# UCL/gp_emulator

Hardware: AMD Instinct MI355X
Metric: test-points/sec for predict(mean+var+grad), N_train=250 D=11 (higher is better)
Workload: dtype f64

## Files before the change

### gp_emulator_amd/csrc/gp_predict_few_kernel.hpp

```cpp
#pragma once
#include "gp_predict_kernel.hpp"

namespace gpk {

constexpr int fkWaves = 8;
constexpr int fkThreads = fkWaves * 64;
constexpr int fkMaxKSteps = 4 * 20;

template <typename T, int D, bool kVar = true>
__global__ __launch_bounds__(fkThreads, 2) void predict_few_kernel(PredictArgs<T> p, int NB) {
  typedef Real<T> R;
  typedef typename R::acc_t acc_t;
  constexpr int DS = row_stride(D);
  constexpr int kVals = D + 2;

  __shared__ __attribute__((aligned(16))) T s_xa[4 * fkMaxKSteps * row_stride(D)];
  __shared__ T s_k[kVar ? fkMaxKSteps : 1][64];
  __shared__ T s_part[fkWaves][kTile][kVals];

  const int tid = threadIdx.x;
  const int lane = tid & 63;
  const int w = __builtin_amdgcn_readfirstlane(tid >> 6);
  const int ml = lane & 15, g = lane >> 4;
  const int n_tiles = (int)((p.M + kTile - 1) / kTile);
  const int e = blockIdx.x / n_tiles, tile = blockIdx.x - e * n_tiles;
  const int NKS = 4 * NB;

  const T* xa = p.xa + e * p.xa_stride;
  const T* frags = p.frags + e * p.frags_stride;
  (void)frags;
  const T* sdp = p.sd + e * p.sd_stride;
  const long long m = (long long)tile * kTile + ml;
  const long long mc = m < p.M ? m : p.M - 1;

  {
    const int n = 16 * NB * DS;
#pragma unroll 4
    for (int i = tid; i < n; i += fkThreads) s_xa[i] = xa[i];
  }

  T t[D];
  T gm = T(0);
#pragma unroll
  for (int d = 0; d < D; ++d) {
    const bool live = d < p.d_actual;
    const int dc = live ? d : p.d_actual - 1;
    const T sc = !live ? T(0) : p.rows_prescaled ? T(1) : sdp[d];
    const T ce = (!live || p.rows_prescaled) ? T(0) : sdp[D + d];
    t[d] = sc * (p.testing[mc * p.d_actual + dc] - ce);
    gm = fma(t[d], t[d], gm);
  }
  gm *= T(-0.5);
  const T poison = gm - gm;
  const T b = sdp[2 * D];
  __syncthreads();

  T mu = T(0);
  T ga[D];
#pragma unroll
  for (int d = 0; d < D; ++d) ga[d] = T(0);
#pragma unroll 1
  for (int ks = w; ks < NKS; ks += fkWaves) {
    const int i = own_index<T>(ks >> 2, ks & 3, g);
    const T* row = &s_xa[i * DS];
    T x[D];
#pragma unroll
    for (int d = 0; d < D; ++d) x[d] = row[d];
    const T al = row[D];
    T k;
    if constexpr (R::kExpand) {
      k = row[D + 1] + gm;
#pragma unroll
      for (int d = 0; d < D; ++d) k = fma(x[d], t[d], k);
      k = R::exp_clamped(k);
    } else {
      T r2 = T(0);
#pragma unroll
      for (int d = 0; d < D; ++d) {
        x[d] -= t[d];
        r2 = fma(x[d], x[d], r2);
      }
      k = b * R::exp_clamped(T(-0.5) * r2);
    }
    if constexpr (kVar) s_k[ks][lane] = k;
    const T wgt = k * al;
    mu += wgt;
#pragma unroll
    for (int d = 0; d < D; ++d) ga[d] = fma(wgt, x[d], ga[d]);
  }
  mu = xor_reduce_groups(mu);
  xor_reduce_groups_n<T, D>(ga);
  if (g == 0) {
    s_part[w][ml][0] = mu;
#pragma unroll
    for (int d = 0; d < D; ++d) s_part[w][ml][1 + d] = ga[d];
  }
  __syncthreads();

  if constexpr (kVar) {
  T vacc = T(0);
  auto column_block = [&](const int J) __attribute__((always_inline)) {
    const T* f = frags + ((size_t)frag_index(J, J, 0, NB) * 64 + lane);
    const int n = 4 * (NB - J);
    acc_t acc = acc_t{T(0), T(0), T(0), T(0)};
    T a_cur[4], a_nxt[4];
#pragma unroll
    for (int s = 0; s < 4; ++s) a_cur[s] = f[(size_t)s * 64];
#pragma unroll 1
    for (int q = 0; q < n; q += 4) {
      const int qn = q + 4 < n ? q + 4 : q;
#pragma unroll
      for (int s = 0; s < 4; ++s) a_nxt[s] = f[(size_t)(qn + s) * 64];
#pragma unroll
      for (int s = 0; s < 4; ++s) acc = R::mfma(a_cur[s], s_k[4 * J + q + s][lane], acc);
#pragma unroll
      for (int s = 0; s < 4; ++s) a_cur[s] = a_nxt[s];
    }
#pragma unroll
    for (int r = 0; r < 4; ++r) vacc = fma(acc[r], s_k[4 * J + r][lane], vacc);
  };
  for (int pr = w; 2 * pr < NB; pr += fkWaves) {
    column_block(pr);
    if (NB - 1 - pr != pr) column_block(NB - 1 - pr);
  }
  vacc = xor_reduce_groups(vacc);
  if (g == 0) s_part[w][ml][1 + D] = vacc;
  __syncthreads();
  }

  if (w == 0 && m < p.M) {
    auto total = [&](const int v) __attribute__((always_inline)) {
      T s = s_part[0][ml][v];
#pragma unroll
      for (int k = 1; k < fkWaves; ++k) s += s_part[k][ml][v];
      return s;
    };
    const T mean = total(0) + poison;
    T* o_mu = p.mu + e * p.M;
    T* o_der = p.deriv + e * p.M * p.d_actual;
    if (g == 0) o_mu[m] = mean;
    if constexpr (kVar) {
      if (g == 1) p.var[e * p.M + m] = b - total(1 + D) + poison;
    }
#pragma unroll
    for (int d = 0; d < D; ++d) {
      if ((d & 3) == g && d < p.d_actual) {
        const T gsum = total(1 + d);
        const T gd = sdp[d] * (R::kExpand ? fma(-t[d], mean, gsum) : gsum + poison);
        if (p.deriv_row_major) o_der[m * p.d_actual + d] = gd;
        else o_der[(long long)d * p.M + m] = gd;
      }
    }
  }
}

}
```

### gp_emulator_amd/csrc/gp_predict_kernel.hpp

```cpp
#pragma once
#include <hip/hip_runtime.h>
#include <stdint.h>
#include <type_traits>
#include <utility>

namespace gpk {

#ifndef GP_WAVES
#define GP_WAVES 8
#endif
#ifndef GP_WAVES_F32
#define GP_WAVES_F32 12
#endif
#ifndef GP_CHUNK
#define GP_CHUNK 64
#endif
#ifndef GP_CHUNK_F32
#define GP_CHUNK_F32 192
#endif
#ifndef GP_ABLATE
#define GP_ABLATE 0
#endif
#ifndef GP_AHEAD
#define GP_AHEAD 4
#endif
#ifndef GP_AHEAD_F32
#define GP_AHEAD_F32 8
#endif
#ifndef GP_RING_PIN
#define GP_RING_PIN 1
#endif
#ifndef GP_MU_DOUBLE
#define GP_MU_DOUBLE 1
#endif
#ifndef GP_ESTRIN
#define GP_ESTRIN 0
#endif
#ifndef GP_EXP_FUSED
#define GP_EXP_FUSED 1
#endif
#ifndef GP_DOTSPLIT
#define GP_DOTSPLIT 1
#endif
#ifndef GP_GROUP_F64
#define GP_GROUP_F64 1
#endif
#ifndef GP_STAMPS
#define GP_STAMPS 0
#endif
constexpr int kTile = 16;
template <typename T, bool kVar = true> struct Geo {
  static constexpr int kWaves = sizeof(T) == 8 ? GP_WAVES : GP_WAVES_F32;
  static constexpr int kThreads = kWaves * 64;
#ifndef GP_WG_PER_CU_SMALL
#define GP_WG_PER_CU_SMALL 0
#endif
  static constexpr int kWGPerCU = kWaves >= 8 ? 1 : (GP_WG_PER_CU_SMALL > 0 ? GP_WG_PER_CU_SMALL : 8 / kWaves);
  static constexpr int kWavesPerSimd = kWaves >= 8 ? kWaves / 4 : kWGPerCU * kWaves / 4;
  static constexpr int kRowsPerWG = kWaves * kTile;
  static constexpr int kChunk = sizeof(T) == 8 ? GP_CHUNK : GP_CHUNK_F32;
};
#ifndef GP_MG_WAVES
#define GP_MG_WAVES 12
#endif
#ifndef GP_MG_WAVES_F32
#define GP_MG_WAVES_F32 16
#endif
#ifndef GP_MG_WG_PER_CU
#define GP_MG_WG_PER_CU 1
#endif
template <typename T> struct Geo<T, false> {
  static constexpr int kWaves = sizeof(T) == 8 ? GP_MG_WAVES : GP_MG_WAVES_F32;
  static constexpr int kThreads = kWaves * 64;
  static constexpr int kWGPerCU = GP_MG_WG_PER_CU;
  static constexpr int kWavesPerSimd = kWGPerCU * kWaves / 4;
  static constexpr int kRowsPerWG = kWaves * kTile;
  static constexpr int kChunk = 1;
};

typedef double f64x4 __attribute__((ext_vector_type(4)));
typedef float f32x4 __attribute__((ext_vector_type(4)));

template <typename F, int... Is>
__device__ __forceinline__ void static_for_impl(F&& f, std::integer_sequence<int, Is...>) {
  (f(std::integral_constant<int, Is>{}), ...);
}
template <int N, typename F>
__device__ __forceinline__ void static_for(F&& f) {
  static_for_impl(f, std::make_integer_sequence<int, N>{});
}

template <typename T> struct Real;
template <> struct Real<double> {
  typedef f64x4 acc_t;
  static constexpr bool kExpand = true;
  static constexpr int kGroup = GP_GROUP_F64;
  __host__ __device__ static constexpr int own_sub(int r, int g) { return 4 * r + g; }
  __device__ static inline acc_t mfma(double a, double b, acc_t c) {
    return __builtin_amdgcn_mfma_f64_16x16x4f64(a, b, c, 0, 0, 0);
  }
  static constexpr double kRoundMagic = 6755399441055744.0;
  __host__ __device__ static inline double exp_(double x) {
#if GP_EXP_FUSED
    const double s = fma(x, 1.4426950408889634, kRoundMagic);
    const double n = s - kRoundMagic;
    const int ni = (int)(unsigned)__builtin_bit_cast(unsigned long long, s);
#else
    x = __builtin_fmax(x, -1000.0);
    const double n = __builtin_rint(x * 1.4426950408889634);
    const int ni = (int)n;
#endif
    double r = fma(n, -6.93147180559945286e-01, x);
    r = fma(n, -2.31904681384629956e-17, r);
#if GP_ESTRIN
    const double r2 = r * r;
    const double p01 = fma(1.00000000000000666e+00, r, 1.0);
    const double p23 = fma(1.66666666665544028e-01, r, 5.00000000000000555e-01);
    const double p45 = fma(8.33333338566834801e-03, r, 4.16666666665732183e-02);
    const double p67 = fma(1.98411702695461072e-04, r, 1.38888889324666632e-03);
    const double p89 = fma(2.76401812311866076e-06, r, 2.48015043709117912e-05);
    const double r4 = r2 * r2;
    const double q0 = fma(r2, p23, p01);
    const double q1 = fma(r2, p67, p45);
    const double q2 = fma(r2, 2.76263485910095559e-07, p89);
    const double r8 = r4 * r4;
    const double s0 = fma(r4, q1, q0);
    const double p = fma(r8, q2, s0);
#else
    double p = 2.76263485910095559e-07;
    p = fma(p, r, 2.76401812311866076e-06);
    p = fma(p, r, 2.48015043709117912e-05);
    p = fma(p, r, 1.98411702695461072e-04);
    p = fma(p, r, 1.38888889324666632e-03);
    p = fma(p, r, 8.33333338566834801e-03);
    p = fma(p, r, 4.16666666665732183e-02);
    p = fma(p, r, 1.66666666665544028e-01);
    p = fma(p, r, 5.00000000000000555e-01);
    p = fma(p, r, 1.00000000000000666e+00);
    p = fma(p, r, 1.0);
#endif
    return ldexp(p, ni);
  }
  __host__ __device__ static inline double exp_clamped(double x) { return exp_(__builtin_fmax(x, -1000.0)); }
  template <int GP>
  __device__ static inline void exp_n(double (&x)[GP]) {
    double n[GP], r[GP], p[GP];
    int ni[GP];
#pragma unroll
    for (int u = 0; u < GP; ++u) x[u] = __builtin_fmax(x[u], -1000.0);
#if GP_EXP_FUSED
#pragma unroll
    for (int u = 0; u < GP; ++u) r[u] = fma(x[u], 1.4426950408889634, kRoundMagic);
#pragma unroll
    for (int u = 0; u < GP; ++u) {
      n[u] = r[u] - kRoundMagic;
      ni[u] = (int)(unsigned)__builtin_bit_cast(unsigned long long, r[u]);
    }
#else
#pragma unroll
    for (int u = 0; u < GP; ++u) {
      n[u] = __builtin_rint(x[u] * 1.4426950408889634);
      ni[u] = (int)n[u];
    }
#endif
#pragma unroll
    for (int u = 0; u < GP; ++u) r[u] = fma(n[u], -6.93147180559945286e-01, x[u]);
#pragma unroll
    for (int u = 0; u < GP; ++u) r[u] = fma(n[u], -2.31904681384629956e-17, r[u]);
#pragma unroll
    for (int u = 0; u < GP; ++u) p[u] = 2.76263485910095559e-07;
    constexpr double c[10] = {2.76401812311866076e-06, 2.48015043709117912e-05, 1.98411702695461072e-04,
                              1.38888889324666632e-03, 8.33333338566834801e-03, 4.16666666665732183e-02,
                              1.66666666665544028e-01, 5.00000000000000555e-01, 1.00000000000000666e+00, 1.0};
#pragma unroll
    for (int j = 0; j < 10; ++j) {
#pragma unroll
      for (int u = 0; u < GP; ++u) p[u] = fma(p[u], r[u], c[j]);
    }
#pragma unroll
    for (int u = 0; u < GP; ++u) x[u] = ldexp(p[u], ni[u]);
  }
  static constexpr double kMaxHalfNorm2 = 67108864.0;
  static constexpr double kFarG = 134217728.0;
};
template <> struct Real<float> {
  typedef f32x4 acc_t;
  static constexpr bool kExpand = false;
#ifndef GP_GROUP_F32
#define GP_GROUP_F32 2
#endif
  static constexpr int kGroup = GP_GROUP_F32;
  __host__ __device__ static constexpr int own_sub(int r, int g) { return 4 * g + r; }
  __device__ static inline acc_t mfma(float a, float b, acc_t c) {
    return __builtin_amdgcn_mfma_f32_16x16x4f32(a, b, c, 0, 0, 0);
  }
  __device__ static inline float exp_(float x) { return __expf(x); }
  __device__ static inline float exp_clamped(float x) { return __expf(x); }
  template <int GP>
  __device__ static inline void exp_n(float (&x)[GP]) {
#pragma unroll
    for (int u = 0; u < GP; ++u) x[u] = __expf(x[u]);
  }
};

template <typename T>
__host__ __device__ constexpr int own_index(int I, int s, int g) {
  return 16 * I + Real<T>::own_sub(s, g);
}

template <typename T>
__host__ __device__ constexpr int point_slot(int n) {
  return 16 * (n / 16) + Real<T>::own_sub((n % 16) / 4, n % 4);
}
template <typename T>
__host__ __device__ constexpr int slot_point(int slot) {
  for (int q = 0; q < 16; ++q)
    if (Real<T>::own_sub(q / 4, q % 4) == slot % 16) return 16 * (slot / 16) + q;
  return -1;
}

struct FragId { int I, J, s; };
__host__ __device__ constexpr int frag_count(int NB) { return NB * (NB + 1) / 2 * 4; }
__host__ __device__ constexpr int frag_col_offset(int J, int NB) { return J * NB - J * (J - 1) / 2; }
__host__ __device__ constexpr FragId frag_at(int n, int NB) {
  const int pair = n >> 2;
  int J = 0;
  while (J + 1 < NB && frag_col_offset(J + 1, NB) <= pair) ++J;
  return FragId{J + pair - frag_col_offset(J, NB), J, n & 3};
}
__host__ __device__ constexpr int frag_index(int I, int J, int s, int NB) {
  return (frag_col_offset(J, NB) + (I - J)) * 4 + s;
}
__host__ __device__ constexpr int frag_count_padded(int NB, int chunk) {
  return (frag_count(NB) + chunk - 1) / chunk * chunk;
}

__host__ __device__ constexpr int row_stride(int D) { return (D + 2 + 3) & ~3; }
#ifndef GP_XA_PAD
#define GP_XA_PAD 1
#endif
template <typename T> __host__ __device__ constexpr int xa_lds_stride(int D) {
  return (GP_XA_PAD && sizeof(T) == 4 && row_stride(D) % 16 == 0) ? row_stride(D) + 4 : row_stride(D);
}

#ifndef GP_FRAG_BUFS
#define GP_FRAG_BUFS 3
#endif
#ifndef GP_FRAG_BUFS_F32
#define GP_FRAG_BUFS_F32 2
#endif
#ifndef GP_SEAM
#define GP_SEAM 2
#endif
constexpr int kLdsBudget = 160 * 1024;
constexpr int kLdsSlack = 32;
template <typename T>
__host__ __device__ constexpr int predict_lds_bytes(int D, int NK, int bufs) {
  const int NP = 16 * ((NK + 3) / 4);
  return (int)sizeof(T) * (NP * xa_lds_stride<T>(D) + bufs * Geo<T>::kChunk * 64 + (2 * D + 1) + 2 * D +
                           2 * Geo<T>::kWaves * kTile * D) + kLdsSlack;
}
template <typename T>
__host__ __device__ constexpr int frag_buffers(int D, int NK) {
  const int want = sizeof(T) == 8 ? GP_FRAG_BUFS : GP_FRAG_BUFS_F32;
  return want > 2 && predict_lds_bytes<T>(D, NK, want) <= kLdsBudget ? want : 2;
}

template <typename T>
struct PredictArgs {
  const T* xa;
  const T* frags;
  const T* sd;
  const T* testing;
  T* mu;
  T* var;
  T* deriv;
  long long M;
  int d_actual;
  int deriv_row_major;
  int n_emulators;
  long long xa_stride, frags_stride, sd_stride;
  unsigned long long* dbg;
  int rows_prescaled;
};

template <int XOR>
__device__ __forceinline__ unsigned swap_halves(unsigned x, unsigned& other) {
  if constexpr (XOR == 16) {
    auto r = __builtin_amdgcn_permlane16_swap(x, x, false, false);
    other = r[1];
    return r[0];
  } else {
    auto r = __builtin_amdgcn_permlane32_swap(x, x, false, false);
    other = r[1];
    return r[0];
  }
}
template <int XOR>
__device__ __forceinline__ float pair_sum(float v) {
  unsigned o, a = swap_halves<XOR>(__float_as_uint(v), o);
  return __uint_as_float(a) + __uint_as_float(o);
}
template <int XOR>
__device__ __forceinline__ double pair_sum(double v) {
  const unsigned long long u = (unsigned long long)__double_as_longlong(v);
  unsigned lo_o, hi_o;
  const unsigned lo_a = swap_halves<XOR>((unsigned)u, lo_o);
  const unsigned hi_a = swap_halves<XOR>((unsigned)(u >> 32), hi_o);
  const double a = __longlong_as_double((long long)(((unsigned long long)hi_a << 32) | lo_a));
  const double o = __longlong_as_double((long long)(((unsigned long long)hi_o << 32) | lo_o));
  return a + o;
}

template <typename T, int N>
__device__ inline void xor_reduce_groups_n(T* v) {
#pragma unroll
  for (int i = 0; i < N; ++i) v[i] = pair_sum<32>(pair_sum<16>(v[i]));
}

template <typename T>
__device__ inline T xor_reduce_groups(T v) {
  return pair_sum<32>(pair_sum<16>(v));
}

template <typename T, int kWaves = Geo<T>::kWaves, int kChunk = Geo<T>::kChunk>
__device__ __forceinline__ void stage_chunk(const T* src, T* dst, int wave, int lane) {
  constexpr int kBytes = kChunk * 64 * (int)sizeof(T);
  constexpr int kPieces = kBytes / 1024;
  static_assert(kPieces * 1024 == kBytes, "chunk must be whole 1 KiB pieces");
  const unsigned voff = (unsigned)lane * 16u;
  const unsigned lds0 = (unsigned)(uintptr_t)(
      (__attribute__((address_space(3))) char*)(reinterpret_cast<char*>(dst)));
#pragma unroll
  for (int pc0 = 0; pc0 < kPieces; pc0 += kWaves) {
    const int pc = pc0 + wave;
    if (pc0 + kWaves <= kPieces || pc < kPieces) {
      const char* s = reinterpret_cast<const char*>(src) + pc * 1024;
      const unsigned m0v = __builtin_amdgcn_readfirstlane(lds0 + pc * 1024);
      unsigned keep;
      asm volatile(
          "s_mov_b32 %0, m0\n\t"
          "s_mov_b32 m0, %1\n\t"
          "s_nop 4\n\t"
          "global_load_lds_dwordx4 %2, %3\n\t"
          "s_mov_b32 m0, %0"
          : "=&s"(keep)
          : "s"(m0v), "v"(voff), "s"(s)
          : "memory");
    }
  }
}
template <typename T, int NP>
__device__ __forceinline__ void stage_pieces(const T* src, T* dst, int first_piece, int lane) {
  const unsigned voff = (unsigned)lane * 16u;
  const unsigned lds0 = (unsigned)(uintptr_t)(
      (__attribute__((address_space(3))) char*)(reinterpret_cast<char*>(dst)));
#pragma unroll
  for (int i = 0; i < NP; ++i) {
    const int pc = first_piece + i;
    const char* s = reinterpret_cast<const char*>(src) + pc * 1024;
    const unsigned m0v = __builtin_amdgcn_readfirstlane(lds0 + pc * 1024);
    unsigned keep;
    asm volatile(
        "s_mov_b32 %0, m0\n\t"
        "s_mov_b32 m0, %1\n\t"
        "s_nop 4\n\t"
        "global_load_lds_dwordx4 %2, %3\n\t"
        "s_mov_b32 m0, %0"
        : "=&s"(keep)
        : "s"(m0v), "v"(voff), "s"(s)
        : "memory");
  }
}
__device__ __forceinline__ void dma_wait() { asm volatile("s_waitcnt vmcnt(0)" ::: "memory"); }

#if GP_STAMPS == 1
#define GP_STAMP(seg)                                                                    \
  do {                                                                                   \
    __builtin_amdgcn_sched_barrier(0);                                                   \
    unsigned long long now_;                                                             \
    asm volatile("s_memtime %0\n\ts_waitcnt lgkmcnt(0)" : "=s"(now_)::"memory");         \
    __builtin_amdgcn_sched_barrier(0);                                                   \
    seg_sum[seg] += now_ - seg_t0;                                                       \
    seg_t0 = now_;                                                                       \
  } while (0)
#else
#define GP_STAMP(seg) do { } while (0)
#endif

template <typename T, int D, int NK, bool kVar = true>
__global__ __launch_bounds__((Geo<T, kVar>::kThreads), (Geo<T, kVar>::kWavesPerSimd)) void predict_kernel(PredictArgs<T> p) {
  typedef Real<T> R;
  typedef Geo<T, kVar> G;
  constexpr int kThreads = G::kThreads;
  constexpr int kRowsPerWG = G::kRowsPerWG;
  typedef typename R::acc_t acc_t;
  constexpr int NB = (NK + 3) / 4;
  constexpr int KL = NK - 4 * (NB - 1);
  constexpr int NP = 16 * NB;
  constexpr int DSG = row_stride(D);
  constexpr int DS = xa_lds_stride<T>(D);
  constexpr int NF = frag_count(NB);
  constexpr int kChunk = G::kChunk;
  constexpr int NCH = (NF + kChunk - 1) / kChunk;
  constexpr int kBufs = kVar ? frag_buffers<T>(D, NK) : 1;
  constexpr int kLook = kBufs - 2;
  constexpr bool kSeamOk = kVar && kBufs == 3 && NCH >= 3 && NCH % 3 == 0;
  constexpr bool kSeamAblated = (GP_ABLATE == 5 || GP_ABLATE == 6) && kSeamOk;
  constexpr bool kSeam = GP_SEAM && !kSeamAblated && kSeamOk;
  constexpr bool kSeamTop = kSeam || kSeamAblated;
  constexpr bool kSeamAlways = kSeam && GP_SEAM == 2;

  __shared__ __attribute__((aligned(16))) T s_xa[NP * DS];
  __shared__ __attribute__((aligned(16))) T s_fr[kBufs][kVar ? kChunk * 64 : 1];
  __shared__ T s_sd[2 * D + 1];
  __shared__ T s_ts[2 * D];
  __shared__ T s_rows[2][G::kWaves][kTile * D];
  static_assert(!kVar || (int)(sizeof(s_xa) + sizeof(s_fr) + sizeof(s_sd) + sizeof(s_ts) + sizeof(s_rows)) + kLdsSlack ==
                             predict_lds_bytes<T>(D, NK, kBufs), "predict_lds_bytes() does not count the kernel's LDS arrays");

  const int tid = threadIdx.x;
  const int lane = tid & 63;
  const int wave = __builtin_amdgcn_readfirstlane(tid >> 6);
  const int ml = lane & 15;
  const int g = lane >> 4;

  const int n_groups = (int)((p.M + kRowsPerWG - 1) / kRowsPerWG);
  int e = 0, cur_e = -1;
  int grp = blockIdx.x;
  while (grp >= n_groups && e < p.n_emulators) { grp -= n_groups; ++e; }

  constexpr int NJ = (kTile * D + 63) / 64;
  auto fetch_rows = [&](int grp_, T (&regs)[NJ]) {
    const long long e0 = ((long long)grp_ * kRowsPerWG + wave * kTile) * p.d_actual;
    const long long emax = p.M * p.d_actual - 1;
#pragma unroll
    for (int j = 0; j < NJ; ++j) {
      long long e_ = e0 + lane + 64 * j;
      e_ = e_ < emax ? e_ : emax;
      regs[j] = p.testing[e_];
    }
  };
  auto stash_rows = [&](int buf_, const T (&regs)[NJ]) {
#pragma unroll
    for (int j = 0; j < NJ; ++j) asm volatile("" ::"v"(regs[j]));
#pragma unroll
    for (int j = 0; j < NJ; ++j)
      if (lane + 64 * j < kTile * p.d_actual) s_rows[buf_][wave][lane + 64 * j] = regs[j];
  };
  int rbuf = 0;
  T rregs[NJ];
  if (e < p.n_emulators) {
    fetch_rows(grp, rregs);
    stash_rows(0, rregs);
  }
#if GP_STAMPS
  unsigned long long seg_sum[8] = {0, 0, 0, 0, 0, 0, 0, 0};
  unsigned long long seg_t0;
  asm volatile("s_memtime %0\n\ts_waitcnt lgkmcnt(0)" : "=s"(seg_t0)::"memory");
#endif

  for (; e < p.n_emulators;) {
    const T* frags = p.frags + e * p.frags_stride;
    auto open_ring = [&]() {
      __syncthreads();
      static_for<1 + kLook>([&](auto cc) {
        constexpr int c = decltype(cc)::value;
        if constexpr (c < NCH) stage_chunk<T, G::kWaves, kChunk>(frags + c * kChunk * 64, &s_fr[c][0], wave, lane);
      });
    };
    if (e != cur_e) {
      cur_e = e;
      if constexpr (kSeamAlways) dma_wait();
      __syncthreads();
      const T* xa = p.xa + e * p.xa_stride;
      for (int i = tid; i < NP * DSG; i += kThreads) s_xa[(i / DSG) * DS + i % DSG] = xa[i];
      const T* sdp = p.sd + e * p.sd_stride;
      if (tid < 2 * D + 1) {
        const bool live = tid == 2 * D || (tid % D) < p.d_actual;
        s_sd[tid] = live ? sdp[tid] : T(0);
        if (tid < 2 * D)
          s_ts[tid] = !live ? T(0) : !p.rows_prescaled ? sdp[tid] : tid < D ? T(1) : T(0);
      }
      if constexpr (!kVar) __syncthreads();
      if constexpr (kVar && kSeamTop) open_ring();
    }
    T* o_mu = p.mu + e * p.M;
    T* o_der = p.deriv + e * p.M * p.d_actual;
    const long long m = (long long)grp * kRowsPerWG + wave * kTile + ml;
    const long long mc = m < p.M ? m : p.M - 1;

    if constexpr (kVar) {
      if constexpr (!kSeamTop) open_ring();
    } else {
      (void)frags;
      __builtin_amdgcn_fence(__ATOMIC_ACQ_REL, "wavefront");
      __builtin_amdgcn_wave_barrier();
    }
    const T b = s_sd[2 * D];
    GP_STAMP(0);

    T t[D];
    T gm = T(0);
    {
      T sdv[D], cv[D], rv[D];
#pragma unroll
      for (int d = 0; d < D; ++d) {
        const int dc = d < p.d_actual ? d : p.d_actual - 1;
        sdv[d] = s_ts[d];
        cv[d] = s_ts[D + d];
        rv[d] = s_rows[rbuf][wave][ml * p.d_actual + dc];
      }
#pragma unroll
      for (int d = 0; d < D; ++d) {
        t[d] = sdv[d] * (rv[d] - cv[d]);
        gm = fma(t[d], t[d], gm);
      }
    }
    gm *= T(-0.5);
    const T poison = gm - gm;
    if constexpr (R::kExpand && GP_EXP_FUSED) {
      const bool in_reach = gm >= T(-R::kFarG);
#pragma unroll
      for (int d = 0; d < D; ++d) t[d] = in_reach ? t[d] : T(0);
      gm = in_reach ? gm : T(-R::kFarG);
    }

    asm volatile("" :: "v"(gm));
    int e_next = e, grp_next = grp + gridDim.x;
    while (grp_next >= n_groups && e_next < p.n_emulators) { grp_next -= n_groups; ++e_next; }
    fetch_rows(e_next < p.n_emulators ? grp_next : grp, rregs);
    const bool ahead = kSeam && e_next == e;

    GP_STAMP(1);
    T kv[NK];
#if GP_MU_DOUBLE
    double mu = 0.0;
#else
    T mu = T(0);
#endif
    T ga[D];
#pragma unroll
    for (int d = 0; d < D; ++d) ga[d] = T(0);

    constexpr int GP = R::kGroup;
    static_for<(NK + GP - 1) / GP>([&](auto qc) {
      constexpr int q0 = decltype(qc)::value * GP;
      constexpr int GU = NK - q0 < GP ? NK - q0 : GP;
      T x[GP][D];
      T al[GP];
      T k[GP];
#pragma unroll
      for (int u = 0; u < GU; ++u) {
        const int q = q0 + u;
        const int i = own_index<T>(q >> 2, q & 3, g);
        const T* row = &s_xa[i * DS];
#pragma unroll
        for (int d = 0; d < D; ++d) x[u][d] = row[d];
        al[u] = row[D];
        if constexpr (R::kExpand) k[u] = row[D + 1] + gm;
      }
#pragma unroll
      for (int u = 0; u < GU; ++u) {
#if GP_ABLATE == 2
        continue;
#endif
        if constexpr (R::kExpand) {
          T part[GP_DOTSPLIT];
          part[0] = k[u];
#pragma unroll
          for (int c = 1; c < GP_DOTSPLIT; ++c) part[c] = T(0);
#pragma unroll
          for (int d = 0; d < D; ++d) part[d % GP_DOTSPLIT] = fma(x[u][d], t[d], part[d % GP_DOTSPLIT]);
#pragma unroll
          for (int c = 1; c < GP_DOTSPLIT; ++c) part[0] += part[c];
          k[u] = part[0];
        } else {
          T r2 = T(0);
#pragma unroll
          for (int d = 0; d < D; ++d) {
            x[u][d] -= t[d];
            r2 = fma(x[u][d], x[u][d], r2);
          }
          k[u] = T(-0.5) * r2;
        }
      }
#pragma unroll
      for (int u = 0; u < GU; ++u) {
#if GP_ABLATE == 2
        k[u] = x[u][0] + t[0];
#else
        k[u] = R::kExpand ? R::exp_(k[u]) : b * R::exp_(k[u]);
#endif
        if constexpr (kVar) kv[q0 + u] = k[u];
      }
#pragma unroll
      for (int u = 0; u < GU; ++u) {
        const T w = k[u] * al[u];
        mu += (decltype(mu))w;
#if GP_ABLATE == 2
        ga[u % D] += w;
#else
#pragma unroll
        for (int d = 0; d < D; ++d) ga[d] = fma(w, x[u][d], ga[d]);
#endif
      }
    });
    GP_STAMP(2);
    const T mu_t = (T)xor_reduce_groups(mu) + poison;
    static_for<(D + 5) / 6>([&](auto bc) {
      constexpr int d0 = decltype(bc)::value * 6;
      constexpr int nb_ = (D - d0 < 6) ? (D - d0) : 6;
      xor_reduce_groups_n<T, nb_>(&ga[d0]);
    });
    {
      T sdv[D];
#pragma unroll
      for (int d = 0; d < D; ++d) sdv[d] = s_sd[d];
#pragma unroll
      for (int d = 0; d < D; ++d)
        ga[d] = R::kExpand ? sdv[d] * fma(-t[d], mu_t, ga[d]) : fma(sdv[d], ga[d], poison);
    }

    if (m < p.M) {
      if (g == 0) o_mu[m] = mu_t;
      int gs = g;
      asm volatile("" : "+v"(gs));
      T gq[(D + 3) / 4];
#pragma unroll
      for (int q = 0; q < (D + 3) / 4; ++q) {
        gq[q] = ga[4 * q];
#pragma unroll
        for (int u = 1; u < 4; ++u)
          if (4 * q + u < D) gq[q] = gs == u ? ga[4 * q + u] : gq[q];
      }
      if (p.deriv_row_major) {
        T* o_row = o_der + m * p.d_actual + gs;
#pragma unroll
        for (int q = 0; q < (D + 3) / 4; ++q)
          if (4 * q + gs < p.d_actual) o_row[4 * q] = gq[q];
      } else {
        T* o_row = o_der + gs * p.M + m;
#pragma unroll
        for (int q = 0; q < (D + 3) / 4; ++q)
          if (4 * q + gs < p.d_actual) o_row[4 * q * p.M] = gq[q];
      }
    }

    GP_STAMP(3);
    stash_rows(rbuf ^ 1, rregs);
    if constexpr (!kVar) {
      rbuf ^= 1;
      e = e_next;
      grp = grp_next;
      continue;
    } else {

    T* o_var = p.var + e * p.M;
    T vacc = T(0);
    acc_t acc;
    constexpr int kAhead = sizeof(T) == 4 ? GP_AHEAD_F32 : GP_AHEAD;
    T afr[kAhead];
#if GP_ABLATE == 1
    static_for<NK>([&](auto qc) { vacc += kv[decltype(qc)::value]; });
    static_for<0>([&](auto fc) {
#else
    static_for<NF>([&](auto fc) {
#endif
      constexpr int f = decltype(fc)::value;
      constexpr int c = f / kChunk, fl = f % kChunk;
      constexpr FragId fid = frag_at(f, NB);
      constexpr int I = fid.I, J = fid.J, s = fid.s;
      if constexpr (fl == 0) {
#if GP_ABLATE == 4
        if constexpr (c == 0) { dma_wait(); __syncthreads(); }
#else
        if constexpr (c == 0 || c + kLook < NCH) {
          dma_wait();
          if constexpr (kLook > 0) {
            if constexpr (c > 0) __builtin_amdgcn_sched_barrier(0);
            asm volatile("s_barrier" ::: "memory");
            if constexpr (c > 0) __builtin_amdgcn_sched_barrier(0);
          } else {
            __syncthreads();
          }
          if constexpr (c + kLook + 1 < NCH) {
            stage_chunk<T, G::kWaves, kChunk>(frags + (c + kLook + 1) * kChunk * 64,
                                              &s_fr[(c + kLook + 1) % kBufs][0], wave, lane);
          } else if constexpr (kSeam && c == NCH - 2) {
            if (kSeamAlways || ahead) stage_chunk<T, G::kWaves, kChunk>(frags, &s_fr[0][0], wave, lane);
          }
        } else if constexpr (GP_ABLATE == 6 && kSeamAblated && c == NCH - 1) {
          __builtin_amdgcn_sched_barrier(0);
          asm volatile("s_barrier" ::: "memory");
          __builtin_amdgcn_sched_barrier(0);
        } else if constexpr (kSeam && c == NCH - 1) {
          if (kSeamAlways || ahead) {
            __builtin_amdgcn_sched_barrier(0);
            asm volatile("s_barrier" ::: "memory");
            __builtin_amdgcn_sched_barrier(0);
            stage_chunk<T, G::kWaves, kChunk>(frags + kChunk * 64, &s_fr[1][0], wave, lane);
          }
        }
#endif
        static_for<kAhead - 1>([&](auto jc) {
          constexpr int n = f + decltype(jc)::value;
          if constexpr (n < NF && (c == 0 || n / kChunk > c - 1 + kLook)) {
#if GP_ABLATE >= 3
            afr[n % kAhead] = kv[n % NK];
#else
            afr[n % kAhead] = s_fr[(n / kChunk) % kBufs][(n % kChunk) * 64 + lane];
#endif
          }
        });
      }
      {
        constexpr int n = f + kAhead - 1;
        if constexpr (n < NF && n / kChunk <= c + kLook) {
#if GP_ABLATE >= 3
          afr[n % kAhead] = kv[(f + 1) % NK];
#else
          afr[n % kAhead] = s_fr[(n / kChunk) % kBufs][(n % kChunk) * 64 + lane];
#endif
        }
      }
      if constexpr (I == J && s == 0) acc = acc_t{T(0), T(0), T(0), T(0)};
      if constexpr (4 * I + s < NK) acc = R::mfma(afr[f % kAhead], kv[4 * I + s], acc);
#if GP_RING_PIN
      if constexpr (sizeof(T) == 4 || GP_RING_PIN > 1) __builtin_amdgcn_sched_barrier(0);
#endif
      if constexpr (I == NB - 1 && s == 3) {
#pragma unroll
        for (int r = 0; r < (J == NB - 1 ? KL : 4); ++r) vacc = fma(acc[r], kv[4 * J + r], vacc);
      }
    });
    rbuf ^= 1;
    GP_STAMP(4);
    vacc = xor_reduce_groups(vacc);
    if (m < p.M && g == 1) o_var[m] = b - vacc + poison;

    e = e_next;
    grp = grp_next;
    GP_STAMP(5);
    }
  }
  if constexpr (kSeamAlways) dma_wait();
#if GP_STAMPS
  if (lane == 0 && p.dbg) {
    for (int k_ = 0; k_ < 8; ++k_) atomicAdd(&p.dbg[k_], seg_sum[k_]);
    atomicAdd(&p.dbg[7], 1ull);
  }
#endif
}

}
```

Baseline: 763.2 million.

## Interleave fragment order across column groups to use independent MFMA accumulators

```diff
diff --git a/gp_emulator_amd/csrc/gp_predict_few_kernel.hpp b/gp_emulator_amd/csrc/gp_predict_few_kernel.hpp
--- a/gp_emulator_amd/csrc/gp_predict_few_kernel.hpp
+++ b/gp_emulator_amd/csrc/gp_predict_few_kernel.hpp
@@ -100,17 +100,19 @@
   if constexpr (kVar) {
   T vacc = T(0);
   auto column_block = [&](const int J) __attribute__((always_inline)) {
-    const T* f = frags + ((size_t)frag_index(J, J, 0, NB) * 64 + lane);
+    auto frag = [&](const int I, const int s) __attribute__((always_inline)) {
+      return frags[(size_t)frag_index(I, J, s, NB) * 64 + lane];
+    };
     const int n = 4 * (NB - J);
     acc_t acc = acc_t{T(0), T(0), T(0), T(0)};
     T a_cur[4], a_nxt[4];
 #pragma unroll
-    for (int s = 0; s < 4; ++s) a_cur[s] = f[(size_t)s * 64];
+    for (int s = 0; s < 4; ++s) a_cur[s] = frag(J, s);
 #pragma unroll 1
     for (int q = 0; q < n; q += 4) {
       const int qn = q + 4 < n ? q + 4 : q;
 #pragma unroll
-      for (int s = 0; s < 4; ++s) a_nxt[s] = f[(size_t)(qn + s) * 64];
+      for (int s = 0; s < 4; ++s) a_nxt[s] = frag(J + qn / 4, s);
 #pragma unroll
       for (int s = 0; s < 4; ++s) acc = R::mfma(a_cur[s], s_k[4 * J + q + s][lane], acc);
 #pragma unroll
diff --git a/gp_emulator_amd/csrc/gp_predict_kernel.hpp b/gp_emulator_amd/csrc/gp_predict_kernel.hpp
--- a/gp_emulator_amd/csrc/gp_predict_kernel.hpp
+++ b/gp_emulator_amd/csrc/gp_predict_kernel.hpp
@@ -219,17 +219,37 @@
   return -1;
 }
 
+#ifndef GP_COLGROUP
+#define GP_COLGROUP 4
+#endif
+#if GP_ABLATE == 7
+constexpr int kColGroup = 1;
+#else
+constexpr int kColGroup = GP_COLGROUP;
+#endif
 struct FragId { int I, J, s; };
 __host__ __device__ constexpr int frag_count(int NB) { return NB * (NB + 1) / 2 * 4; }
 __host__ __device__ constexpr int frag_col_offset(int J, int NB) { return J * NB - J * (J - 1) / 2; }
+__host__ __device__ constexpr int frag_group_width(int J0, int NB) { return NB - J0 < kColGroup ? NB - J0 : kColGroup; }
+__host__ __device__ constexpr int frag_row_width(int I, int J0, int NB) {
+  return I - J0 + 1 < frag_group_width(J0, NB) ? I - J0 + 1 : frag_group_width(J0, NB);
+}
+__host__ __device__ constexpr int frag_row_offset(int I, int J0, int NB) {
+  const int d = I - J0, w = frag_group_width(J0, NB);
+  return d <= w ? d * (d + 1) / 2 : w * (w + 1) / 2 + (d - w) * w;
+}
+__host__ __device__ constexpr int frag_index(int I, int J, int s, int NB) {
+  const int J0 = J - J % kColGroup;
+  return (frag_col_offset(J0, NB) + frag_row_offset(I, J0, NB)) * 4 + s * frag_row_width(I, J0, NB) + (J - J0);
+}
 __host__ __device__ constexpr FragId frag_at(int n, int NB) {
   const int pair = n >> 2;
-  int J = 0;
-  while (J + 1 < NB && frag_col_offset(J + 1, NB) <= pair) ++J;
-  return FragId{J + pair - frag_col_offset(J, NB), J, n & 3};
-}
-__host__ __device__ constexpr int frag_index(int I, int J, int s, int NB) {
-  return (frag_col_offset(J, NB) + (I - J)) * 4 + s;
+  int J0 = 0;
+  while (J0 + kColGroup < NB && frag_col_offset(J0 + kColGroup, NB) <= pair) J0 += kColGroup;
+  int I = J0;
+  while (I + 1 < NB && frag_col_offset(J0, NB) + frag_row_offset(I + 1, J0, NB) <= pair) ++I;
+  const int r = n - (frag_col_offset(J0, NB) + frag_row_offset(I, J0, NB)) * 4, w = frag_row_width(I, J0, NB);
+  return FragId{I, J0 + r % w, r / w};
 }
 __host__ __device__ constexpr int frag_count_padded(int NB, int chunk) {
   return (frag_count(NB) + chunk - 1) / chunk * chunk;
@@ -658,7 +678,11 @@
 
     T* o_var = p.var + e * p.M;
     T vacc = T(0);
-    acc_t acc;
+    constexpr int kAcc = GP_ABLATE == 7 ? GP_COLGROUP : kColGroup;
+    acc_t acc[kAcc];
+#if GP_ABLATE == 7
+    static_for<kAcc>([&](auto ac) { acc[decltype(ac)::value] = acc_t{T(0), T(0), T(0), T(0)}; });
+#endif
     constexpr int kAhead = sizeof(T) == 4 ? GP_AHEAD_F32 : GP_AHEAD;
     T afr[kAhead];
 #if GP_ABLATE == 1
@@ -724,14 +748,27 @@
 #endif
         }
       }
-      if constexpr (I == J && s == 0) acc = acc_t{T(0), T(0), T(0), T(0)};
-      if constexpr (4 * I + s < NK) acc = R::mfma(afr[f % kAhead], kv[4 * I + s], acc);
+      constexpr int J0 = J - J % kColGroup, GW = frag_group_width(J0, NB);
+      constexpr int a = GP_ABLATE == 7 ? f % kAcc : J - J0;
+      if constexpr (I == J && s == 0) acc[a] = acc_t{T(0), T(0), T(0), T(0)};
+      if constexpr (4 * I + s < NK) acc[a] = R::mfma(afr[f % kAhead], kv[4 * I + s], acc[a]);
 #if GP_RING_PIN
       if constexpr (sizeof(T) == 4 || GP_RING_PIN > 1) __builtin_amdgcn_sched_barrier(0);
 #endif
-      if constexpr (I == NB - 1 && s == 3) {
-#pragma unroll
-        for (int r = 0; r < (J == NB - 1 ? KL : 4); ++r) vacc = fma(acc[r], kv[4 * J + r], vacc);
+      if constexpr (I == NB - 1 && s == 3 && J == J0 + GW - 1) {
+#if GP_ABLATE == 7
+        static_for<kAcc>([&](auto ac) {
+          constexpr int a_ = decltype(ac)::value;
+#pragma unroll
+          for (int r = 0; r < (J == NB - 1 ? KL : 4); ++r) vacc = fma(acc[a_][r], kv[4 * J + r], vacc);
+        });
+#else
+        static_for<GW>([&](auto jc) {
+          constexpr int Jc = J0 + decltype(jc)::value;
+#pragma unroll
+          for (int r = 0; r < (Jc == NB - 1 ? KL : 4); ++r) vacc = fma(acc[Jc - J0][r], kv[4 * Jc + r], vacc);
+        });
+#endif
       }
     });
     rbuf ^= 1;
```

Result: no change. 759.3 million (-0.5%).
